# Jarvis73/PEMP

Hardware: AMD Instinct MI355X
Metric: episodes/sec (PEMP stage-1 eval step, PASCAL-5i-shaped 1-shot, ResNet-50) (higher is better)
Workload: dtype f32

## Files before the change

pemp_amd/build.py:

```python
import hashlib
import os
import subprocess
from concurrent.futures import ThreadPoolExecutor

HERE = os.path.dirname(os.path.abspath(__file__))
CSRC = os.path.join(HERE, "csrc")
OBJ = os.path.join(HERE, "_obj")
OUT = os.path.join(HERE, "libpemp_hip.so")
SOURCES = ("conv_igemm.hip", "conv_dma.hip", "conv_dma2.hip", "conv_panel.hip", "conv_stem_pool.hip", "conv_wgrad.hip", "train_ops.hip", "pool_misc.hip", "head.hip", "head_bwd.hip", "cedt.hip",
           "episode_io.hip", "dropout.hip", "cm_linear.hip", "pfenet.hip", "pfenet_bwd.hip", "canet.hip", "canet_bwd.hip", "rpmms.hip", "rpmms_bwd.hip")
FLAGS = ["-O3", "--offload-arch=gfx950", "-std=c++17", "-fPIC"]


def _headers():
    return [os.path.join(CSRC, f) for f in sorted(os.listdir(CSRC)) if f.endswith((".h", ".inc"))] + \
           [os.path.join(HERE, "..", "include", "pemp_hip.h")]


def csrc_digest():
    h = hashlib.sha1()
    for f in sorted(os.listdir(CSRC)):
        with open(os.path.join(CSRC, f), "rb") as fh:
            h.update(f.encode() + b"\0" + fh.read())
    with open(os.path.join(HERE, "..", "include", "pemp_hip.h"), "rb") as fh:
        h.update(fh.read())
    return h.hexdigest()[:12]


CONV_ENGINE = ("common.h", "conv_common.h", "conv_tiles.h", "conv_igemm.hip", "conv_dma.hip", "conv_dma2.hip", "conv_panel.hip", "conv_stem_pool.hip")


def conv_digest():
    h = hashlib.sha1()
    for f in CONV_ENGINE:
        with open(os.path.join(CSRC, f), "rb") as fh:
            h.update(f.encode() + b"\0" + fh.read())
    return h.hexdigest()[:12]


def needs_build():
    if not os.path.exists(OUT):
        return True
    t = os.path.getmtime(OUT)
    deps = [os.path.join(CSRC, f) for f in os.listdir(CSRC)] + [os.path.join(HERE, "..", "include", "pemp_hip.h")]
# ... 49 lines not shown
```

pemp_amd/csrc/conv_common.h:

```cpp
#pragma once
#include "common.h"

namespace pemp {

typedef __attribute__((ext_vector_type(16))) float f32x16;
typedef __attribute__((ext_vector_type(4))) float v4f;
typedef __attribute__((ext_vector_type(8))) __bf16 bf16x8;
typedef __attribute__((ext_vector_type(2))) unsigned int u32x2;

#define PEMP_CONV_BF16_IO 0x100u

__device__ __forceinline__ v4f load_quad(const float* base, size_t off, unsigned bf16) {
    if (!bf16) return *(const v4f*)(base + off);
    const u32x2 r = *(const u32x2*)((const unsigned short*)base + off);
    return v4f{__builtin_bit_cast(float, r.x << 16), __builtin_bit_cast(float, r.x & 0xFFFF0000u),
               __builtin_bit_cast(float, r.y << 16), __builtin_bit_cast(float, r.y & 0xFFFF0000u)};
}

__device__ __forceinline__ unsigned int bf16_bits(float f) {
    const unsigned int u = __builtin_bit_cast(unsigned int, f);
    if ((u & 0x7FFFFFFFu) > 0x7F800000u) return (u >> 16) | 0x40u;
    return (u + 0x7FFFu + ((u >> 16) & 1u)) >> 16;
}

// ... 300 lines not shown
int conv_dma2_hybrid_rows(int M, int Cout);
int launch_conv_dma2_bf16(int shape, const ConvArgs& a, hipStream_t st);
int launch_conv_dma2_db(int shape, ConvArgs a, void* ws, size_t ws_bytes, bool split, hipStream_t st);
struct SplitKPlan { int full, split, pieces; size_t ws_bytes; };
SplitKPlan conv_dma2_splitk_plan(int shape, const ConvArgs& a);
int launch_conv_dma2_splitk(int shape, ConvArgs a, void* ws, size_t ws_bytes, hipStream_t st);
int launch_conv_dma2_split3(int shape, ConvArgs a, void* ws, size_t ws_bytes, bool split, hipStream_t st);
int launch_conv_dma2_group_split3(int shape, ConvGroupArgs& g, hipStream_t st);
int launch_conv_dma2_split3_stats(int shape, const ConvArgs& a, hipStream_t st);
bool conv_dma2_split3_stats_shape(int shape);
int launch_conv_dma2_split3_persist(int shape, const ConvArgs& a, hipStream_t st);
bool conv_dma2_persist_out_split3(int shape);
int launch_conv_dma2_split3_pre(int shape, bool persistent, const ConvArgs& a, hipStream_t st);
bool conv_panel_supported(const ConvArgs& a);
int launch_conv_panel(int shape, const ConvArgs& a, hipStream_t st);
int conv_dma2_simds();
int pack_split3(const float* w, void* out, int cout, int kpad, hipStream_t st);
int launch_conv_stem_pool(const ConvArgs& a, hipStream_t st);
int conv_stem_pool_out(int i);

}
```

pemp_amd/csrc/conv_igemm.hip:

```cpp
#include "conv_tiles.h"

namespace pemp {


template <int BM, int BN, int WGM, bool STEM>
__global__ __launch_bounds__(256) void conv_igemm_kernel(ConvArgs a) {
    constexpr int WGN = 4 / WGM;
    constexpr int WM = BM / WGM, WN = BN / WGN;
    constexpr int TM = WM / 32, TN = WN / 32;
    constexpr int AL = BM / 32, BL = BN / 32;
    static_assert(TM >= 1 && TN >= 1, "wave tile");

    extern __shared__ __attribute__((aligned(16))) v4f smem[];
    v4f* As = smem;
    v4f* Bs = smem + 2 * 8 * BM;

    const int tid = threadIdx.x;
    const int lane = tid & 63;
    const int wave = tid >> 6;
    const int wm0 = (wave / WGN) * WM;
    const int wn0 = (wave % WGN) * WN;
    const int lr = lane & 31, lh = lane >> 5;

    const int ntn = a.Cout / BN;
// ... 292 lines not shown
                     "conv2d: PEMP_CONV_POOL3S2 needs PEMP_CONV_STEM4 with split3 weights (a tile id 41..49), no residual, no padding value");
        return launch_conv_stem_pool(a, (hipStream_t)stream);
    }
    PEMP_REQUIRE(tile != 33 && tile != 53, "conv2d: no split-K variant of the 64 x 64 tile");
    PEMP_REQUIRE(tile != 45 && tile != 55, "conv2d: no split3 form of the 128 x 64 8-wave tile");
    PEMP_REQUIRE(tile != 48, "conv2d: no persistent split3 form of the 128 x 128 4-wave tile");
    PEMP_REQUIRE(t.exists, "conv2d: unknown tile id %d", tile);
    hipStream_t st = (hipStream_t)stream;
    PEMP_REQUIRE(t.presplit == ((d->flags & PEMP_CONV_IN_SPLIT3) != 0), "conv2d: tile ids 146 / 149 and PEMP_CONV_IN_SPLIT3 come together (tile %d)", tile);
    if (t.presplit) {
        PEMP_REQUIRE(!stem && !ws && a.ntaps > 1 && a.ntaps <= 16 && a.ldx == a.Cin && !(d->flags & PEMP_CONV_SHIFT_PER_IMAGE),
                     "conv2d: tile %d takes convs of 2..16 taps with ldx == Cin, no per-image shift, no workspace", tile);
        PEMP_REQUIRE(conv_dma2_supported(a) && (long long)a.Cout * a.Kpad * 6 < (1ll << 31),
                     "conv2d: tile %d needs <= 32 taps and operands < 2 GiB (a padding value behind the activations)", tile);
        PEMP_REQUIRE_COUT("conv2d", t.shape, a.Cout);
        return launch_conv_dma2_split3_pre(t.shape, t.persistent, a, st);
    }
    if (t.family == TILE_SPLIT3) {
        PEMP_REQUIRE(!stem && conv_dma2_supported(a) && (long long)a.Cout * a.Kpad * 6 < (1ll << 31),
                     "conv2d: split3 tile %d needs a geometry of the buffer-addressed kernels (no stem, <= 32 taps, operands < 2 GiB)", tile);
        PEMP_REQUIRE_COUT("conv2d", t.shape, a.Cout);
        if (t.panel) {
            PEMP_REQUIRE(!ws && conv_panel_supported(a),
                         "conv2d: tile %d needs a 1x1 conv without padding, Kpad <= 256, no padding value / per-image shift / workspace, operands < 2 GiB", tile);
            return launch_conv_panel(t.shape, a, st);
        }
        if (t.persistent && (!out_split3 || conv_dma2_persist_out_split3(t.shape))) return launch_conv_dma2_split3_persist(t.shape, a, st);
        return launch_conv_dma2_split3(t.shape, a, ws, ws_bytes, t.splitk, st);
    }
    if (t.family == TILE_DMA2 && t.splitk) {
// ... 252 lines not shown
```

pemp_amd/csrc/conv_tiles.h:

```cpp
#pragma once
#include <initializer_list>
#include "conv_common.h"

namespace pemp {

struct TileShape { int bm, bn, wgm, nw, wgm3; };
inline constexpr TileShape kTileShapes[10] = {
    {0, 0, 0, 0, 0},
    {128, 128, 2, 4, 4},
    {128, 64, 2, 4, 4},
    {64, 64, 2, 4, 2},
    {128, 128, 4, 8, 4},
    {128, 64, 4, 8, 0},
    {256, 128, 4, 8, 8},
    {256, 256, 4, 8, 0},
    {32, 64, 2, 4, 0},
    {64, 64, 2, 4, 0},
};

template <int S, bool S3 = false>
struct Tile {
    static constexpr int BM = kTileShapes[S].bm, BN = kTileShapes[S].bn, NW = kTileShapes[S].nw;
    static constexpr int WGM = S3 ? kTileShapes[S].wgm3 : kTileShapes[S].wgm;
};
// ... 24 lines not shown
            if (shape == S) return f(Tile<S, Fam::s3>{});
        }
        return with_tile<Fam, S + 1>(shape, f);
    }
}

enum TileFamily { TILE_NONE = 0, TILE_IGEMM, TILE_DMA, TILE_DMA2, TILE_SPLIT3 };
struct TileId {
    int family;
    int shape;
    bool splitk;
    bool persistent;
    bool exists;
    bool panel;
    bool presplit;
};

inline TileId decode_tile(int id) {
    TileId t = {TILE_NONE, 0, false, false, false, false, false};
    const int decade = id / 10, s = id % 10;
    if (id == 146 || id == 149) {
        t.family = TILE_SPLIT3, t.shape = 6, t.exists = t.presplit = true, t.persistent = id == 149;
        return t;
    }
    if (decade == 7 && in_family<FamPanel>(s)) {
        t.family = TILE_SPLIT3, t.shape = s, t.exists = t.panel = true;
        return t;
    }
    if (id < 1 || id > 56 || s == 0) return t;
    t.shape = s;
    if (decade == 0) t.family = TILE_IGEMM, t.exists = in_family<FamIgemm>(s);
    else if (decade == 1) t.family = TILE_DMA, t.exists = in_family<FamFp32>(s);
    else if (decade == 2) t.family = TILE_DMA2, t.exists = true;
    else if (decade == 3) t.family = TILE_DMA2, t.splitk = true, t.exists = in_family<FamSplitK>(s);
    else if (decade == 4 && (s == 7 || s == 9)) t.family = TILE_SPLIT3, t.persistent = t.exists = true, t.shape = s == 7 ? 3 : 6;
    else if (decade == 4) t.family = TILE_SPLIT3, t.exists = in_family<FamSplit3>(s);
    else t.family = TILE_SPLIT3, t.splitk = true, t.exists = in_family<FamSplit3>(s) && in_family<FamSplitK>(s);
// ... 45 lines not shown
```

pemp_amd/ops.py:

```python
import ctypes as C
import collections
import functools
import json
import os

import torch

from . import _lib
from ._lib import ConvDesc, CONV_RELU, CONV_SHIFT_PER_IMAGE, CONV_STEM4, CONV_POOL3S2, CONV_OUT_SPLIT3, CONV_IN_SPLIT3, CONV_OUT_SPLIT3_ALSO


def _stream():
    return C.c_void_p(torch.cuda.current_stream().cuda_stream)


def _p(t):
    return C.c_void_p(t.data_ptr()) if t is not None else C.c_void_p(0)


def _chk_dev(*ts):
    for t in ts:
        if t is not None and (not t.is_cuda):
            raise _lib.PempHipError("pemp_amd ops need device (cuda/HIP) tensors; there is no CPU path")

# ... 32 lines not shown
           8: (32, 64),
           9: (64, 64)}
Tile = collections.namedtuple("Tile", "shape family splitk persistent_of")
SPLIT3_PERSISTENT = {47: 43, 49: 46}
TILES = {base + s: Tile(_SHAPES[s], family, base in (30, 50), None)
         for family, base, shapes in (("igemm", 0, (1, 2, 3)),
                                      ("dma", 10, range(1, 8)),
                                      ("dma2", 20, range(1, 10)),
                                      ("dma2", 30, (1, 2, 4, 5, 6, 7)),
                                      ("split3", 40, (1, 2, 3, 4, 6)),
                                      ("split3", 50, (1, 2, 4, 6)))
         for s in shapes}
TILES.update({t: TILES[of]._replace(persistent_of=of) for t, of in SPLIT3_PERSISTENT.items()})
TILES.update({70 + s: Tile(_SHAPES[s], "split3", False, None) for s in (1, 2)})
TILES.update({146: Tile(_SHAPES[6], "split3", False, None), 149: Tile(_SHAPES[6], "split3", False, 146)})
_NO_TILE = Tile(None, None, False, None)


def tile_shape(t):
    return TILES.get(t, _NO_TILE).shape


TILE_VARIANTS = {t: TILES[t].shape for t in (13, 14, 12, 11, 15, 3, 17, 16, 23, 24, 22, 21, 25, 27, 26, 28, 29)}
SPLIT3_TILES = (43, 42, 41, 44, 46, 47, 49)
SPLIT3_SPLITK_TILES = (51, 52, 54, 56)
SPLIT3_DEFAULT_TILE = 43
SPLIT3_PANEL_TILES = (71, 72)
SPLIT3_PANEL = os.environ.get("PEMP_SPLIT3_PANEL", "1") != "0"
SPLIT3_PRESPLIT_TILES = (146, 149)
SPLIT3_PRESPLIT = os.environ.get("PEMP_SPLIT3_PRESPLIT", "1") != "0"
AUTOTUNE = True
PICK_HOOK = None
SPLITK = os.environ.get("PEMP_CONV_SPLITK", "1") != "0"
DEFAULT_TILE = 13
_TILE_CACHE = {}
_TILE_CACHE_FILE = os.environ.get("PEMP_TILE_CACHE")
WGRAD_PICKS = {}
if _TILE_CACHE_FILE and os.path.exists(_TILE_CACHE_FILE):
    with open(_TILE_CACHE_FILE) as _f:
        for _k, _v in json.load(_f).items():
            _key = json.loads(_k)
            if _key and _key[0] == "wgrad":
                WGRAD_PICKS[tuple(_key[1:])] = tuple(_v) if isinstance(_v, list) else int(_v)
            else:
                _TILE_CACHE[tuple(_key)] = int(_v)
# ... 95 lines not shown
    best = min(top, key=lambda t: final[t])
    _TILE_CACHE[key] = best
    save_picks()
    return best


def _tile_bn(t):
    return TILES[t].shape[1]


def _panel_ok(p, n, ho, wo, ldx, ldy, ldr, h, w, pad_value, splitk, per_image_shift):
    lim = 1 << 31
    return (SPLIT3_PANEL and PICK_HOOK is None and p.kh == 1 and p.kw == 1 and p.pad == 0 and p.kpad <= 256 and p.cin % 32 == 0
            and pad_value is None and not splitk and not per_image_shift and n * h * w * ldx * 4 < lim
            and n * ho * wo * max(ldy, ldr) * 4 < lim)


def pack_split3(w):
    co, kpad = w.shape
    if w.dtype != torch.float32 or not w.is_contiguous() or kpad % 32:
        raise ValueError("pack_split3: a contiguous fp32 [Cout, Kpad] with Kpad % 32 == 0")
    out = torch.empty((co, kpad // 32, 3, 32), dtype=torch.bfloat16, device=w.device)
    _lib.check(_lib.load().pemp_pack_split3_bf16(_p(w), _p(out), co, kpad, _stream()), "pemp_pack_split3_bf16")
    return out


def hybrid_rows(n, ho, wo, cout):
    d = ConvDesc(n, ho, wo, 32, 32, ho, wo, cout, cout, 1, 1, 1, 0, 1, 0, 32, 0, 29)
    return int(_lib.load().pemp_conv2d_hybrid_rows(C.byref(d)))

# ... 60 lines not shown

def conv2d(x, p, out=None, residual=None, shift_override=None, per_image_shift=False, relu=None, tile=0,
           pad_value=None, splitk=False, dropblock=None, out_split3=False, x_split3=False, also_split3=None):
    if out_split3 or x_split3:
        what = "a pre-split output" if out_split3 else "a pre-split input"
        if p.w3 is None or p.stem:
            raise ValueError(f"conv2d: {what} needs a split3 layer (ConvParams.w3), not the fp32 chain or a stem")
        if splitk or dropblock is not None:
            raise ValueError(f"conv2d: {what} has no split-K / DropBlock form")
        if out_split3 and tile and (tile not in SPLIT3_TILES + SPLIT3_PRESPLIT_TILES):
            raise ValueError(f"conv2d: a pre-split output needs an unsplit split3 tile id, got {tile}")
        if x_split3 and (p.kh * p.kw == 1 or per_image_shift or p.cin % 32 or p.cout % 128):
            raise ValueError("conv2d: a pre-split input needs a multi-tap conv with Cin % 32 == 0 and Cout % 128 == 0, no per-image shift")
    if also_split3 is not None and (not x_split3 or out_split3 or residual is not None):
        raise ValueError("conv2d: a second, pre-split output needs a pre-split input (x_split3), no out_split3, no residual")
    if (tile in SPLIT3_PRESPLIT_TILES) != bool(x_split3) and (tile or not x_split3):
        raise ValueError(f"conv2d: the tile ids {SPLIT3_PRESPLIT_TILES} and x_split3 come together (tile {tile})")
    if x.dtype == torch.bfloat16 and not x_split3:
        return _conv2d_bf16(x, p, out, residual, shift_override, per_image_shift, relu, tile, pad_value)
    n, h, w, cin, ldx, ho, wo, out, ldy, ldr = _conv_geom("conv2d", x, p, out, residual, x_split3=x_split3, out_split3=out_split3)
    if also_split3 is not None and _split3_dims(also_split3, "also_split3") != (n, ho, wo, p.cout):
        raise ValueError(f"conv2d: also_split3 shape {tuple(also_split3.shape)} != {split3_shape(n, ho, wo, p.cout)}")
    lib = _lib.load()
    _chk_dev(x, p.w, out, residual, also_split3)
    if also_split3 is not None:
        residual = also_split3
    shift = p.shift if shift_override is None else shift_override
    if pad_value is not None:
        _chk_dev(pad_value)
        if x_split3:
            if tuple(pad_value.shape) != (cin // 32, 3, 32) or pad_value.dtype != torch.bfloat16 or not pad_value.is_contiguous():
                raise ValueError(f"conv2d: with x_split3, pad_value must be a contiguous bf16 [{cin // 32}, 3, 32] split vector")
# ... 45 lines not shown
            ws, ws_bytes = _splitk_ws(lib, d, x.device)
            _check_sk(lib, lib.pemp_conv2d_splitk_nhwc_f32(C.byref(d), _p(x), _p(pw), _p(out), _p(p.scale), _p(shift), _p(residual),
                                                           C.c_void_p(ws), ws_bytes, _stream()), ws, "pemp_conv2d_splitk_nhwc_f32")
        elif pad_value is None:
            _lib.check(lib.pemp_conv2d_nhwc_f32(C.byref(d), _p(x), _p(pw), _p(out), _p(p.scale), _p(shift),
                                                _p(residual), _stream()), "pemp_conv2d_nhwc_f32")
        else:
            _lib.check(lib.pemp_conv2d_padv_nhwc_f32(C.byref(d), _p(x), _p(pw), _p(out), _p(p.scale), _p(shift),
                                                     _p(residual), _p(pad_value), _stream()), "pemp_conv2d_padv_nhwc_f32")

    if tile == 0:
        key = (p.cin, p.cout, p.kh, p.kw, p.stride, p.pad, p.dil, (6 if dropblock is not None else 4) if splitk else int(p.stem) + (7 if dropblock is not None else 0),
               n, h, w, int(residual is not None and also_split3 is None), int(pad_value is not None)) + ((3,) if s3 else ())
        if x_split3 or out_split3:
            key += (146,) * int(x_split3) + (17,) * int(out_split3) + (64,) * int(also_split3 is not None)
            cands = lambda: _fits(list(SPLIT3_PRESPLIT_TILES if x_split3 else SPLIT3_TILES), p.cout)
        elif s3:
            panel = _panel_ok(p, n, ho, wo, ldx, ldy, ldr, h, w, pad_value, splitk, per_image_shift)
            if panel:
                key += (71,)
            cands = lambda: _fits(list(SPLIT3_TILES) + (list(SPLIT3_SPLITK_TILES) if splitk else []) +
                                  (list(SPLIT3_PANEL_TILES) if panel else []), p.cout)
        else:
            def cands():
                ids = list(GROUP_TILES if dropblock is not None else TILE_VARIANTS) + (list(SPLITK_TILES) if splitk else [])
                if 29 in ids and not (hybrid_rows(n, ho, wo, p.cout) and dma2_supported(x, p)):
                    ids.remove(29)
                return _fits(ids, p.cout)
        tile = _choose_tile(key, n * ho * wo, launch, cands,
                            SPLIT3_PRESPLIT_TILES[0] if x_split3 else SPLIT3_DEFAULT_TILE if s3 else DEFAULT_TILE + (10 if dropblock is not None else 0))
    launch(tile)
# ... 819 lines not shown
```

scratch/conv_trace_layers.py:

```python
import collections
import csv
import sys

trace, per_step = sys.argv[1], int(sys.argv[2])
steps = int(sys.argv[3]) if len(sys.argv) > 3 else 20
rows = sorted(csv.DictReader(open(trace)), key=lambda r: int(r["Start_Timestamp"]))
conv = [r for r in rows if any(k in r["Kernel_Name"] for k in ("conv_dma", "conv_igemm", "conv_stem_pool", "conv_panel"))][-steps * per_step:]
dur = lambda r: (int(r["End_Timestamp"]) - int(r["Start_Timestamp"])) / 1e3
pos = collections.defaultdict(list)
for i, r in enumerate(conv):
    pos[i % per_step].append(r)
print(f"conv launches per step {per_step}, steps {steps}: conv {sum(map(dur, conv)) / steps / 1e3:.3f} ms per step")
print(f"{'pos':>3} {'mean us':>9} {'grid':>8} {'wg':>4}  kernel")
for p in range(per_step):
    rs = pos[p]
    r = rs[-1]
    name = r["Kernel_Name"].split("(")[0].replace("void pemp::", "").replace("pemp::", "")
    g = r.get("Grid_Size", r.get("Grid_Size_X", "")); wg = r.get("Workgroup_Size", r.get("Workgroup_Size_X", ""))
    print(f"{p:>3} {sum(map(dur, rs)) / len(rs):9.1f} {g:>8} {wg:>4}  {name}")
```

scratch/s3_layers_bench.py:

```python
import argparse
import hashlib
import os
import sys

import torch

sys.path.insert(0, os.path.dirname(os.path.dirname(os.path.abspath(__file__))))
from pemp_amd import ops

UNSPLIT = (43, 42, 41, 44, 46, 47, 49)
SPLIT = (52, 51, 54, 56)
PANEL = ops.SPLIT3_PANEL_TILES
PRESPLIT = ops.SPLIT3_PRESPLIT_TILES
LAYERS = ((256, 1024, 1, 1, True, False), (512, 1024, 1, 1, False, False), (1024, 256, 1, 1, False, False),
          (256, 256, 3, 2, False, False), (128, 512, 1, 1, True, False), (1024, 512, 1, 1, False, False),
          (256, 256, 3, 2, False, True),
          (64, 256, 1, 1, True, False, 1, 101), (64, 256, 1, 1, False, False, 1, 101), (256, 512, 1, 1, False, False, 2, 101),
          (128, 128, 3, 1, False, False), (128, 128, 3, 1, False, False, 2, 101), (64, 64, 3, 1, False, False, 1, 101),
          (512, 128, 1, 1, False, False),
          (256, 256, 3, 12, False, True))


def timed(fn, reps, n=5):
    for _ in range(2):
        fn()
    e0, e1 = torch.cuda.Event(enable_timing=True), torch.cuda.Event(enable_timing=True)
    best, worst = 1e9, 0.0
    for _ in range(reps):
# ... 60 lines not shown
                continue
            run = lambda: ops.conv2d(x, prm, residual=res, pad_value=pad_value, out=out, tile=tile)
            run()
            same = torch.equal(out, ref)
            if tile in SPLIT:
                hashes.append(f"{tile}=" + ("43" if same else digest(out)))
            us, worst = timed(run, args.reps)
            mark = "" if same else (" ~" if tile in SPLIT else " !")
            cells.append(f"{tile}: {us:7.1f}..{worst:6.1f}us {fl / us / 1e6:5.1f}TF{mark}")
            if tile not in SPLIT and not same:
                hashes.append(f"{tile}=MISMATCH:{digest(out)}")
        if k > 1 and cout % 128 == 0:
            sbuf = torch.zeros((M + 4) * cin * 3, dtype=torch.bfloat16, device=dev)
            sbuf[:(M + 1) * cin * 3] = presplit(buf[:M + 1]).reshape(-1)
            xs, pvs = sbuf[:M * cin * 3].view(N, HW, HW, cin // 32, 3, 32), sbuf[M * cin * 3:(M + 1) * cin * 3].view(cin // 32, 3, 32)
            for tile in keep(PRESPLIT):
                run = lambda: ops.conv2d(xs, prm, residual=res, pad_value=pvs if padv else None, out=out, tile=tile, x_split3=True)
                run()
                same = torch.equal(out, ref)
                us, worst = timed(run, args.reps)
                cells.append(f"{tile}: {us:7.1f}..{worst:6.1f}us {fl / us / 1e6:5.1f}TF{'' if same else ' !'}")
            if not has_res:
                want = presplit(ref)
                outs = torch.empty_like(want)
                for tile in keep(PRESPLIT):
                    run = lambda: ops.conv2d(xs, prm, pad_value=pvs if padv else None, out=out, tile=tile, x_split3=True, also_split3=outs)
                    out.zero_()
                    run()
                    same = torch.equal(out, ref) and torch.equal(outs.view(torch.int16), want.view(torch.int16))
                    us, worst = timed(run, args.reps)
                    cells.append(f"{tile}+s: {us:7.1f}..{worst:6.1f}us{'' if same else ' !'}")
                del want, outs
            del sbuf, xs, pvs
        if k == 1 and not has_res:
            want = presplit(ref)
            outs = torch.empty_like(want)
            for tile in keep((43, 42, 41, 44, 46, 47, 49) if not args.ids else ()):
                if cout % ops._tile_bn(tile):
                    continue
                run = lambda: ops.conv2d(x, prm, out=outs, tile=tile, out_split3=True)
                run()
                same = torch.equal(outs.view(torch.int16), want.view(torch.int16))
                us, worst = timed(run, args.reps)
                cells.append(f"{tile}s: {us:7.1f}..{worst:6.1f}us{'' if same else ' !'}")
            del want, outs
        print(f"{name:>16} k{k} d{dil} res{int(has_res)} | " + " | ".join(cells), flush=True)
        print(f"{'':>16} hash " + " ".join(hashes), flush=True)
    print("(146 / 149: on the pre-split input; NNs: id NN writing a pre-split output, ! = not the split of id 43's;")
    print(" NNN+s: id NNN writing fp32 and the pre-split copy, ! = either differs)")
    print("(! = an unsplit id differs from id 43; ~ = a split-K id differs from id 43, expected where it splits)")


if __name__ == "__main__":
    main()
```

Before: 1485.

## Add row-staged 3x3 conv kernel reusing one activation stage across kw taps

Adds a new split3 conv kernel (tiles 246/249) for 3x3 stride-1 convs on pre-split bf16 input. It stages a contiguous band of up to 288 input rows per kernel row and reads the three kw taps from that same LDS stage via shifted indices, instead of loading one stage per tap. This is meant to cut global-to-LDS traffic and barriers per K step. The autotuner adds these tiles as candidates when the shape fits, at the cost of more LDS use and a more complex pipeline schedule.

After: 1506, median of 6. +1.4%, better.

```diff
diff --git a/pemp_amd/build.py b/pemp_amd/build.py
--- a/pemp_amd/build.py
+++ b/pemp_amd/build.py
@@ -7,7 +7,7 @@
 CSRC = os.path.join(HERE, "csrc")
 OBJ = os.path.join(HERE, "_obj")
 OUT = os.path.join(HERE, "libpemp_hip.so")
-SOURCES = ("conv_igemm.hip", "conv_dma.hip", "conv_dma2.hip", "conv_panel.hip", "conv_stem_pool.hip", "conv_wgrad.hip", "train_ops.hip", "pool_misc.hip", "head.hip", "head_bwd.hip", "cedt.hip",
+SOURCES = ("conv_igemm.hip", "conv_dma.hip", "conv_dma2.hip", "conv_panel.hip", "conv_row3.hip", "conv_stem_pool.hip", "conv_wgrad.hip", "train_ops.hip", "pool_misc.hip", "head.hip", "head_bwd.hip", "cedt.hip",
            "episode_io.hip", "dropout.hip", "cm_linear.hip", "pfenet.hip", "pfenet_bwd.hip", "canet.hip", "canet_bwd.hip", "rpmms.hip", "rpmms_bwd.hip")
 FLAGS = ["-O3", "--offload-arch=gfx950", "-std=c++17", "-fPIC"]
 
@@ -27,7 +27,7 @@
     return h.hexdigest()[:12]
 
 
-CONV_ENGINE = ("common.h", "conv_common.h", "conv_tiles.h", "conv_igemm.hip", "conv_dma.hip", "conv_dma2.hip", "conv_panel.hip", "conv_stem_pool.hip")
+CONV_ENGINE = ("common.h", "conv_common.h", "conv_tiles.h", "conv_igemm.hip", "conv_dma.hip", "conv_dma2.hip", "conv_panel.hip", "conv_row3.hip", "conv_stem_pool.hip")
 
 
 def conv_digest():
diff --git a/pemp_amd/csrc/conv_common.h b/pemp_amd/csrc/conv_common.h
--- a/pemp_amd/csrc/conv_common.h
+++ b/pemp_amd/csrc/conv_common.h
@@ -338,6 +338,8 @@
 int launch_conv_dma2_split3_pre(int shape, bool persistent, const ConvArgs& a, hipStream_t st);
 bool conv_panel_supported(const ConvArgs& a);
 int launch_conv_panel(int shape, const ConvArgs& a, hipStream_t st);
+bool conv_row3_supported(const ConvArgs& a);
+int launch_conv_row3(bool persistent, const ConvArgs& a, hipStream_t st);
 int conv_dma2_simds();
 int pack_split3(const float* w, void* out, int cout, int kpad, hipStream_t st);
 int launch_conv_stem_pool(const ConvArgs& a, hipStream_t st);
diff --git a/pemp_amd/csrc/conv_igemm.hip b/pemp_amd/csrc/conv_igemm.hip
--- a/pemp_amd/csrc/conv_igemm.hip
+++ b/pemp_amd/csrc/conv_igemm.hip
@@ -330,6 +330,12 @@
         PEMP_REQUIRE(conv_dma2_supported(a) && (long long)a.Cout * a.Kpad * 6 < (1ll << 31),
                      "conv2d: tile %d needs <= 32 taps and operands < 2 GiB (a padding value behind the activations)", tile);
         PEMP_REQUIRE_COUT("conv2d", t.shape, a.Cout);
+        if (t.row3) {
+            PEMP_REQUIRE(conv_row3_supported(a),
+                         "conv2d: tile %d unsupported: needs a 3x3 / stride 1 / pad == dil conv, the plain fp32 output without residual / padding value, "
+                         "and a stage of at most 288 rows (256 + 2 d + d ceil((255 + 2 d) / W))", tile);
+            return launch_conv_row3(t.persistent, a, st);
+        }
         return launch_conv_dma2_split3_pre(t.shape, t.persistent, a, st);
     }
     if (t.family == TILE_SPLIT3) {
diff --git a/pemp_amd/csrc/conv_row3.hip b/pemp_amd/csrc/conv_row3.hip
--- /dev/null
+++ b/pemp_amd/csrc/conv_row3.hip
@@ -0,0 +1,481 @@
+#include "conv_tiles.h"
+
+namespace pemp {
+
+typedef __attribute__((address_space(3))) void* lptr_t;
+
+constexpr int ROW3_BM = 256, ROW3_BN = 128, ROW3_NW = 8, ROW3_WGM = 4;
+constexpr int ROW3_SR = 288;
+constexpr int ROW3_AQ = ROW3_SR * 12, ROW3_BQ = ROW3_BN * 12;
+constexpr int ROW3_AL = (ROW3_AQ + ROW3_NW * 64 - 1) / (ROW3_NW * 64);
+constexpr int ROW3_BL = ROW3_BQ / (ROW3_NW * 64);
+constexpr int ROW3_SPARE = ROW3_AL * ROW3_NW * 64 - ROW3_AQ;
+static_assert(ROW3_BQ % (ROW3_NW * 64) == 0 && ROW3_SPARE % 64 == 0 && ROW3_SPARE < ROW3_NW * 64, "whole waves in the last A round");
+constexpr size_t row3_lds() { return (size_t)(2 * ROW3_AQ + 2 * ROW3_BQ + ROW3_SPARE) * sizeof(v4f); }
+static_assert(row3_lds() <= 160 * 1024, "LDS of a CU");
+
+constexpr int row3_a_tail(int ph) { return ph == 2 ? 3 : ph == 0 ? ROW3_AL - 3 : 0; }
+constexpr int row3_a_first(int ph) { return ph == 0 ? 3 : 0; }
+static_assert(row3_a_tail(0) + row3_a_tail(1) + row3_a_tail(2) == ROW3_AL, "a group's pieces over its window");
+constexpr int row3_behind(int ph) { return ph == 2 ? 0 : row3_a_tail((ph + 2) % 3); }
+constexpr int row3_behind_first() { return ROW3_BL + row3_a_tail(2); }
+
+__global__ __launch_bounds__(ROW3_NW * 64) __attribute__((amdgpu_waves_per_eu(2))) void conv_row3_kernel(ConvArgs a) {
+#if defined(__HIP_DEVICE_COMPILE__)
+    constexpr int BM = ROW3_BM, BN = ROW3_BN, NW = ROW3_NW, WGM = ROW3_WGM, WGN = NW / WGM;
+    constexpr int WM = BM / WGM, WN = BN / WGN, TM = WM / 32, TN = WN / 32;
+    constexpr int AL = ROW3_AL, BL = ROW3_BL;
+    constexpr int NMF = 6 * TM * TN, NDS = 3 * TM + 3 * TN;
+
+    extern __shared__ __attribute__((aligned(16))) v4f smem[];
+    v4f* As = smem;
+    v4f* Bs = smem + 2 * ROW3_AQ;
+    v4f* Sp = Bs + 2 * ROW3_BQ;
+
+    const int tid = threadIdx.x;
+    const int lane = tid & 63;
+    const int wave = __builtin_amdgcn_readfirstlane(tid >> 6);
+    const int wm0 = (wave / WGN) * WM, wn0 = (wave % WGN) * WN;
+    const int lr = lane & 31, lh = lane >> 5;
+
+    const int ntn = a.Cout / BN;
+    const int tile_id = xcd_tile_order(blockIdx.x, gridDim.x);
+    const int m0 = (tile_id / ntn) * BM, n0 = (tile_id % ntn) * BN;
+
+    const int d = a.dil, W = a.W, Wd = W + d;
+    const int f0 = m0 - d;
+    const int R0 = f0 >= 0 ? f0 / W : -((W - 1 - f0) / W);
+    const int c0 = f0 - R0 * W;
+    const int rowb = a.ldx * 6;
+    const __amdgpu_buffer_rsrc_t rx =
+        __builtin_amdgcn_make_buffer_rsrc((void*)((const char*)a.x - (ptrdiff_t)(d * W + d) * rowb), 0, 0x80000000u, 0x00020000);
+    const __amdgpu_buffer_rsrc_t rw = __builtin_amdgcn_make_buffer_rsrc((void*)a.w, 0, 0x80000000u, 0x00020000);
+
+    unsigned a_voff[AL], a_ok = 0, b_voff[BL];
+#pragma unroll
+    for (int i = 0; i < AL; ++i) {
+        const int q = i * NW * 64 + tid, srow = q / 12, pos = q - srow * 12;
+        const int src = (pos & ~3) | ((pos & 3) ^ ((srow >> 2) & 3));
+        const int t = srow + c0, rr = t / Wd, cc = t - rr * Wd;
+        const int f = (R0 + rr) * W + cc;
+        const bool pix = srow < ROW3_SR && cc < W && f >= 0 && f < a.M && f < m0 + BM + d;
+        const int h = pix ? (R0 + rr) % a.H : 0;
+        a_voff[i] = (unsigned)((f + d) * rowb + src * 16);
+#pragma unroll
+        for (int kh = 0; kh < 3; ++kh)
+            if (pix && (unsigned)(h + (kh - 1) * d) < (unsigned)a.H) a_ok |= 1u << (3 * i + kh);
+    }
+#pragma unroll
+    for (int i = 0; i < BL; ++i) {
+        const int q = i * NW * 64 + tid, row = q / 12, pos = q - row * 12;
+        const int src = (pos & ~3) | ((pos & 3) ^ ((row >> 2) & 3));
+        b_voff[i] = (unsigned)((n0 + row) * a.Kpad * 6 + src * 16);
+    }
+    const int taph = d * W * rowb;
+    const int NG = 3 * a.cin_steps, nkl = a.nk;
+
+#define PEMP_ROW3_DMA_A(i_, ab_, cb_, kh_, ok_)                                                                   \
+    do {                                                                                                          \
+        const int so_ = __builtin_amdgcn_readfirstlane((kh_) * taph + (cb_) * 192);                              \
+        const bool in_ = (((a_ok & (0u - (unsigned)(ok_))) >> (3 * (i_) + (kh_))) & 1u) != 0u;    \
+        v4f* dst_ = As + (ab_) * ROW3_AQ + (i_) * NW * 64 + wave * 64;                                            \
+        if ((i_) == AL - 1 && ROW3_SPARE) dst_ = wave * 64 < NW * 64 - ROW3_SPARE ? dst_ : Sp + (wave * 64 - (NW * 64 - ROW3_SPARE)); \
+        __builtin_amdgcn_raw_ptr_buffer_load_lds(rx, (lptr_t)dst_, 16, in_ ? a_voff[i_] : 0x80000000u, so_, 0, 0); \
+    } while (0)
+#define PEMP_ROW3_DMA_B(bb_, cb_, tap_, ok_)                                                                      \
+    do {                                                                                                          \
+        const int so_ = __builtin_amdgcn_readfirstlane(((tap_) * a.Cin + (cb_) * 32) * 6);                       \
+        _Pragma("unroll") for (int i = 0; i < BL; ++i)                                                            \
+            __builtin_amdgcn_raw_ptr_buffer_load_lds(rw, (lptr_t)(Bs + (bb_) * ROW3_BQ + i * NW * 64 + wave * 64), 16, \
+                                                     (ok_) ? b_voff[i] : 0x80000000u, so_, 0, 0);                 \
+    } while (0)
+
+    int aidx[TM][3][2];
+#pragma unroll
+    for (int mi = 0; mi < TM; ++mi) {
+        const int m = m0 + wm0 + mi * 32 + lr;
+        const int s = m - f0 + d * (m / W - R0);
+#pragma unroll
+        for (int kw = 0; kw < 3; ++kw) {
+            const int row = s + (kw - 1) * d, sw = (row >> 2) & 3;
+            aidx[mi][kw][0] = row * 12 + (lh ^ sw);
+            aidx[mi][kw][1] = row * 12 + ((2 + lh) ^ sw);
+        }
+    }
+    const int brow3 = (wn0 + lr) * 12, bsw3 = (lr >> 2) & 3;
+
+    f32x16 acc[TM][TN];
+#pragma unroll
+    for (int mi = 0; mi < TM; ++mi)
+#pragma unroll
+        for (int ni = 0; ni < TN; ++ni)
+#pragma unroll
+            for (int e = 0; e < 16; ++e) acc[mi][ni][e] = 0.f;
+    v4f aq3[2][TM][3], bf3[2][TN][3];
+
+#define PEMP_ROW3_READ(dst_, ab_, bb_, kw_, j_)                                                                   \
+    do {                                                                                                          \
+        const v4f* Ab_ = As + (ab_) * ROW3_AQ;                                                                    \
+        const v4f* Bb_ = Bs + (bb_) * ROW3_BQ;                                                                    \
+        const int pb_ = (2 * (j_) + lh) ^ bsw3;                                                                   \
+        _Pragma("unroll") for (int mi = 0; mi < TM; ++mi)                                                         \
+            _Pragma("unroll") for (int pl = 0; pl < 3; ++pl)                                                      \
+                aq3[dst_][mi][pl] = Ab_[aidx[mi][kw_][j_] + pl * 4];                                              \
+        _Pragma("unroll") for (int ni = 0; ni < TN; ++ni)                                                         \
+            _Pragma("unroll") for (int pl = 0; pl < 3; ++pl)                                                      \
+                bf3[dst_][ni][pl] = Bb_[brow3 + ni * 32 * 12 + pl * 4 + pb_];                                     \
+    } while (0)
+
+#define PEMP_ROW3_MMA(src_)                                                                                       \
+    do {                                                                                                          \
+        _Pragma("unroll") for (int mi = 0; mi < TM; ++mi) _Pragma("unroll") for (int ni = 0; ni < TN; ++ni) {     \
+            const bf16x8 ah_ = __builtin_bit_cast(bf16x8, aq3[src_][mi][0]);                                      \
+            const bf16x8 am_ = __builtin_bit_cast(bf16x8, aq3[src_][mi][1]);                                      \
+            const bf16x8 al_ = __builtin_bit_cast(bf16x8, aq3[src_][mi][2]);                                      \
+            const bf16x8 bh_ = __builtin_bit_cast(bf16x8, bf3[src_][ni][0]);                                      \
+            const bf16x8 bm_ = __builtin_bit_cast(bf16x8, bf3[src_][ni][1]);                                      \
+            const bf16x8 bl_ = __builtin_bit_cast(bf16x8, bf3[src_][ni][2]);                                      \
+            acc[mi][ni] = __builtin_amdgcn_mfma_f32_32x32x16_bf16(al_, bh_, acc[mi][ni], 0, 0, 0);                \
+            acc[mi][ni] = __builtin_amdgcn_mfma_f32_32x32x16_bf16(ah_, bl_, acc[mi][ni], 0, 0, 0);                \
+            acc[mi][ni] = __builtin_amdgcn_mfma_f32_32x32x16_bf16(am_, bm_, acc[mi][ni], 0, 0, 0);                \
+            acc[mi][ni] = __builtin_amdgcn_mfma_f32_32x32x16_bf16(am_, bh_, acc[mi][ni], 0, 0, 0);                \
+            acc[mi][ni] = __builtin_amdgcn_mfma_f32_32x32x16_bf16(ah_, bm_, acc[mi][ni], 0, 0, 0);                \
+            acc[mi][ni] = __builtin_amdgcn_mfma_f32_32x32x16_bf16(ah_, bh_, acc[mi][ni], 0, 0, 0);                \
+        }                                                                                                         \
+    } while (0)
+
+#define PEMP_ROW3_STEP(PH_, GG_, OKB_, OKA1_, OKA2_)                                                              \
+    do {                                                                                                          \
+        const int ab = (GG_) & 1, bb_ = ((GG_) + (PH_)) & 1;                                                      \
+        PEMP_ROW3_READ(1, ab, bb_, PH_, 1);                                                                       \
+        __builtin_amdgcn_sched_barrier(0);                                                                        \
+        PEMP_ROW3_MMA(0);                                                                                         \
+        __builtin_amdgcn_sched_barrier(0);                                                                        \
+         \
+        __builtin_amdgcn_s_waitcnt(0xC07F);              \
+        asm volatile("s_waitcnt vmcnt(%0) lgkmcnt(0)" ::"n"(row3_behind(PH_)) : "memory");                        \
+        __builtin_amdgcn_s_barrier();                                                        \
+        __builtin_amdgcn_sched_barrier(0);                                                                        \
+        if ((PH_) == 2) PEMP_ROW3_READ(0, ab ^ 1, bb_ ^ 1, 0, 0);                                                 \
+        else PEMP_ROW3_READ(0, ab, bb_ ^ 1, (PH_) + 1, 0);                                                        \
+        if ((PH_) == 0) PEMP_ROW3_DMA_B(bb_, cb, kh * 3 + 2, OKB_);                                               \
+        else PEMP_ROW3_DMA_B(bb_, cbn, khn * 3 + (PH_) - 1, OKB_);                                                \
+        _Pragma("unroll") for (int i = 0; i < row3_a_tail(PH_); ++i) {                                            \
+            if ((PH_) == 2) PEMP_ROW3_DMA_A(row3_a_first(PH_) + i, ab, cbn2, khn2, OKA2_);                        \
+            else PEMP_ROW3_DMA_A(row3_a_first(PH_) + i, ab ^ 1, cbn, khn, OKA1_);                                 \
+        }                                                                                                         \
+        PEMP_ROW3_MMA(1);                \
+        _Pragma("unroll") for (int k_ = 0; k_ < NMF; ++k_) {                                                      \
+            __builtin_amdgcn_sched_group_barrier(0x008, 1, 0);                                                    \
+            if (k_ < NDS) __builtin_amdgcn_sched_group_barrier(0x100, 1, 0);                                      \
+            else if (k_ < NDS + BL + row3_a_tail(PH_)) __builtin_amdgcn_sched_group_barrier(0x020, 1, 0);         \
+        }                                                                                                         \
+        __builtin_amdgcn_sched_barrier(0);                                                                        \
+    } while (0)
+    static_assert(NDS + BL + ROW3_AL <= NMF, "one LDS read / one DMA per MFMA slot");
+
+#pragma unroll
+    for (int i = 0; i < AL; ++i) PEMP_ROW3_DMA_A(i, 0, 0, 0, true);
+    PEMP_ROW3_DMA_B(0, 0, 0, true);
+    PEMP_ROW3_DMA_B(1, 0, 1, true);
+#pragma unroll
+    for (int i = 0; i < row3_a_tail(2); ++i) PEMP_ROW3_DMA_A(i, 1, 0, 1, true);
+    asm volatile("s_waitcnt vmcnt(%0)" ::"n"(row3_behind_first()) : "memory");
+    __builtin_amdgcn_s_barrier();
+    __builtin_amdgcn_sched_barrier(0);
+
+    PEMP_ROW3_READ(0, 0, 0, 0, 0);
+    int cb = 0, kh = 0;
+    for (int g = 0; g < NG; ++g) {
+        const int cbn = kh == 2 ? cb + 1 : cb, khn = kh == 2 ? 0 : kh + 1;
+        const int cbn2 = khn == 2 ? cbn + 1 : cbn, khn2 = khn == 2 ? 0 : khn + 1;
+        PEMP_ROW3_STEP(0, g, 3 * g + 2 < nkl, g + 1 < NG, false);
+        PEMP_ROW3_STEP(1, g, 3 * g + 3 < nkl, false, false);
+        PEMP_ROW3_STEP(2, g, 3 * g + 4 < nkl, false, g + 2 < NG);
+        cb = cbn;
+        kh = khn;
+    }
+
+    __builtin_amdgcn_s_waitcnt(0xC07F);
+    asm volatile("s_waitcnt vmcnt(0) lgkmcnt(0)" ::: "memory");
+    __builtin_amdgcn_s_barrier();
+    __builtin_amdgcn_sched_barrier(0);
+    static_assert(NW * 1024 * sizeof(float) <= 2 * ROW3_AQ * sizeof(v4f), "one 4 KB transpose patch per wave");
+    conv_epilogue_lds<TM, TN>(a, acc, (float*)smem + wave * 1024, m0 + wm0, n0 + wn0, lane);
+#endif
+}
+
+template <int TM, int TN>
+__device__ __forceinline__ void conv_row3_epilogue(const ConvArgs& a, f32x16 (&acc)[TM][TN], float* S, int m_base, int n_base, int lane,
+                                                   const v4f (&scv)[TN], const v4f (&shv)[TN]) {
+    const bool relu = a.flags & PEMP_CONV_RELU;
+    const int lr = lane & 31, lh = lane >> 5;
+    const int rr = lane >> 3, c4 = (lane & 7) * 4;
+#pragma unroll
+    for (int ni = 0; ni < TN; ++ni) {
+        const int n = n_base + ni * 32 + c4;
+        const v4f sc = scv[ni], sh = shv[ni];
+#pragma unroll
+        for (int mi = 0; mi < TM; ++mi) {
+#pragma unroll
+            for (int e = 0; e < 16; ++e) S[((e & 3) + 8 * (e >> 2) + 4 * lh) * 32 + lr] = acc[mi][ni][e];
+            asm volatile("s_waitcnt lgkmcnt(0)" ::: "memory");
+#pragma unroll
+            for (int i = 0; i < 4; ++i) {
+                const int row = rr + 8 * i;
+                const int m = m_base + mi * 32 + row;
+                const v4f v = *(const v4f*)(S + row * 32 + c4);
+                if (m < a.M) {
+                    const v4f add = sh;
+                    v4f o;
+                    o.x = __builtin_fmaf(v.x, sc.x, add.x);
+                    o.y = __builtin_fmaf(v.y, sc.y, add.y);
+                    o.z = __builtin_fmaf(v.z, sc.z, add.z);
+                    o.w = __builtin_fmaf(v.w, sc.w, add.w);
+                    if (relu) {
+                        o.x = fmaxf(o.x, 0.f);
+                        o.y = fmaxf(o.y, 0.f);
+                        o.z = fmaxf(o.z, 0.f);
+                        o.w = fmaxf(o.w, 0.f);
+                    }
+                    store_quad(a.y, (size_t)m * a.ldy + n, o, 0);
+                }
+            }
+            asm volatile("s_waitcnt lgkmcnt(0)" ::: "memory");
+        }
+    }
+}
+
+__global__ __launch_bounds__(ROW3_NW * 64) __attribute__((amdgpu_waves_per_eu(2))) void conv_row3p_kernel(ConvArgs a) {
+#if defined(__HIP_DEVICE_COMPILE__)
+    constexpr int BM = ROW3_BM, BN = ROW3_BN, NW = ROW3_NW, WGM = ROW3_WGM, WGN = NW / WGM;
+    constexpr int WM = BM / WGM, WN = BN / WGN, TM = WM / 32, TN = WN / 32;
+    constexpr int AL = ROW3_AL, BL = ROW3_BL;
+    constexpr int NMF = 6 * TM * TN, NDS = 3 * TM + 3 * TN;
+    constexpr int NST = TM * TN * 4;
+    static_assert(row3_behind_first() + NST <= 63, "vmcnt range");
+
+    extern __shared__ __attribute__((aligned(16))) v4f smem[];
+    v4f* As = smem;
+    v4f* Bs = smem + 2 * ROW3_AQ;
+    v4f* Sp = Bs + 2 * ROW3_BQ;
+
+    const int tid = threadIdx.x;
+    const int lane = tid & 63;
+    const int wave = __builtin_amdgcn_readfirstlane(tid >> 6);
+    const int wm0 = (wave / WGN) * WM, wn0 = (wave % WGN) * WN;
+    const int lr = lane & 31, lh = lane >> 5;
+
+    const int ntn = a.Cout / BN;
+    const int T = (a.M + BM - 1) / BM * ntn;
+    const int xcd = (int)blockIdx.x & 7, idx = (int)blockIdx.x >> 3;
+    const int q8 = T >> 3, r8 = T & 7;
+    const int t_first = xcd < r8 ? xcd * (q8 + 1) : r8 * (q8 + 1) + (xcd - r8) * q8;
+    const int t_cnt = q8 + (xcd < r8 ? 1 : 0);
+    const int gx = ((int)gridDim.x - xcd + 7) >> 3;
+    if (idx >= t_cnt) return;
+    int j = idx;
+    int m0 = ((t_first + j) / ntn) * BM, n0 = ((t_first + j) % ntn) * BN;
+
+    const int d = a.dil, W = a.W, Wd = W + d;
+    const int rowb = a.ldx * 6;
+    const __amdgpu_buffer_rsrc_t rx =
+        __builtin_amdgcn_make_buffer_rsrc((void*)((const char*)a.x - (ptrdiff_t)(d * W + d) * rowb), 0, 0x80000000u, 0x00020000);
+    const __amdgpu_buffer_rsrc_t rw = __builtin_amdgcn_make_buffer_rsrc((void*)a.w, 0, 0x80000000u, 0x00020000);
+
+    unsigned a_voff[AL], a_ok = 0, b_voff[BL];
+    auto a_offsets = [&](const int m0_, const bool ok_) {
+        const int f0 = m0_ - d;
+        const int R0 = f0 >= 0 ? f0 / W : -((W - 1 - f0) / W);
+        const int c0 = f0 - R0 * W;
+        a_ok = 0;
+#pragma unroll
+        for (int i = 0; i < AL; ++i) {
+            const int q = i * NW * 64 + tid, srow = q / 12, pos = q - srow * 12;
+            const int src = (pos & ~3) | ((pos & 3) ^ ((srow >> 2) & 3));
+            const int t = srow + c0, rr = t / Wd, cc = t - rr * Wd;
+            const int f = (R0 + rr) * W + cc;
+            const bool pix = ok_ && srow < ROW3_SR && cc < W && f >= 0 && f < a.M && f < m0_ + BM + d;
+            const int h = pix ? (R0 + rr) % a.H : 0;
+            a_voff[i] = (unsigned)((f + d) * rowb + src * 16);
+#pragma unroll
+            for (int kh = 0; kh < 3; ++kh)
+                if (pix && (unsigned)(h + (kh - 1) * d) < (unsigned)a.H) a_ok |= 1u << (3 * i + kh);
+        }
+    };
+    auto b_offsets = [&](const int n0_, const bool ok_) {
+#pragma unroll
+        for (int i = 0; i < BL; ++i) {
+            const int q = i * NW * 64 + tid, row = q / 12, pos = q - row * 12;
+            const int src = (pos & ~3) | ((pos & 3) ^ ((row >> 2) & 3));
+            b_voff[i] = ok_ ? (unsigned)((n0_ + row) * a.Kpad * 6 + src * 16) : 0x80000000u;
+        }
+    };
+    int aidx[TM][3][2];
+    auto reader = [&](const int m0_) {
+        const int f0 = m0_ - d;
+        const int R0 = f0 >= 0 ? f0 / W : -((W - 1 - f0) / W);
+#pragma unroll
+        for (int mi = 0; mi < TM; ++mi) {
+            const int m = m0_ + wm0 + mi * 32 + lr;
+            const int s = m - f0 + d * (m / W - R0);
+#pragma unroll
+            for (int kw = 0; kw < 3; ++kw) {
+                const int row = s + (kw - 1) * d, sw = (row >> 2) & 3;
+                aidx[mi][kw][0] = row * 12 + (lh ^ sw);
+                aidx[mi][kw][1] = row * 12 + ((2 + lh) ^ sw);
+            }
+        }
+    };
+    a_offsets(m0, true);
+    b_offsets(n0, true);
+    const int taph = d * W * rowb;
+    const int NG = 3 * a.cin_steps, ncb = a.cin_steps;
+    const int brow3 = (wn0 + lr) * 12, bsw3 = (lr >> 2) & 3;
+    const int c4_ = (lane & 7) * 4;
+    v4f aq3[2][TM][3], bf3[2][TN][3];
+
+#pragma unroll
+    for (int i = 0; i < AL; ++i) PEMP_ROW3_DMA_A(i, 0, 0, 0, true);
+    PEMP_ROW3_DMA_B(0, 0, 0, true);
+    PEMP_ROW3_DMA_B(1, 0, 1, true);
+#pragma unroll
+    for (int i = 0; i < row3_a_tail(2); ++i) PEMP_ROW3_DMA_A(i, 1, 0, 1, true);
+    asm volatile("s_waitcnt vmcnt(%0)" ::"n"(row3_behind_first()) : "memory");
+    __builtin_amdgcn_s_barrier();
+    __builtin_amdgcn_sched_barrier(0);
+
+    int gg = 0;
+    int cb = 0, kh = 0;
+    for (;;) {
+        f32x16 acc[TM][TN];
+#pragma unroll
+        for (int mi = 0; mi < TM; ++mi)
+#pragma unroll
+            for (int ni = 0; ni < TN; ++ni)
+#pragma unroll
+                for (int e = 0; e < 16; ++e) acc[mi][ni][e] = 0.f;
+        const int jn = j + gx;
+        const bool more = jn < t_cnt;
+        const int m0n = more ? ((t_first + jn) / ntn) * BM : m0, n0n = more ? ((t_first + jn) % ntn) * BN : n0;
+        reader(m0);
+
+        PEMP_ROW3_READ(0, gg & 1, gg & 1, 0, 0);
+#define PEMP_ROW3_NEXT_GROUPS()                                                                                   \
+        int cbn = kh == 2 ? cb + 1 : cb;                                                                          \
+        const int khn = kh == 2 ? 0 : kh + 1;                                                                     \
+        cbn = cbn == ncb ? 0 : cbn;                                                                               \
+        int cbn2 = khn == 2 ? cbn + 1 : cbn;                                                                      \
+        const int khn2 = khn == 2 ? 0 : khn + 1;                                                                  \
+        cbn2 = cbn2 == ncb ? 0 : cbn2
+        for (int g = 0; g < NG - 1; ++g, ++gg) {
+            PEMP_ROW3_NEXT_GROUPS();
+            PEMP_ROW3_STEP(0, gg, true, true, true);
+            if (g == NG - 2) a_offsets(m0n, more);
+            PEMP_ROW3_STEP(1, gg, true, true, true);
+            PEMP_ROW3_STEP(2, gg, true, true, true);
+            cb = cbn;
+            kh = khn;
+        }
+        const int abl = gg & 1;
+        {
+            PEMP_ROW3_NEXT_GROUPS();
+            PEMP_ROW3_STEP(0, gg, true, true, true);
+            b_offsets(n0n, more);
+            PEMP_ROW3_STEP(1, gg, true, true, true);
+            PEMP_ROW3_READ(1, abl, (gg + 2) & 1, 2, 1);
+            __builtin_amdgcn_sched_barrier(0);
+            PEMP_ROW3_MMA(0);
+            __builtin_amdgcn_sched_barrier(0);
+            __builtin_amdgcn_s_waitcnt(0xC07F);
+            asm volatile("s_waitcnt lgkmcnt(0)" ::: "memory");
+            __builtin_amdgcn_s_barrier();
+            __builtin_amdgcn_sched_barrier(0);
+            PEMP_ROW3_MMA(1);
+            __builtin_amdgcn_sched_barrier(0);
+            cb = cbn;
+            kh = khn;
+            (void)cbn2;
+            (void)khn2;
+            ++gg;
+        }
+#undef PEMP_ROW3_NEXT_GROUPS
+        v4f scv[TN], shv[TN];
+#pragma unroll
+        for (int ni = 0; ni < TN; ++ni) {
+            const int n = n0 + wn0 + ni * 32 + c4_;
+            scv[ni] = a.scale ? *(const v4f*)(a.scale + n) : v4f{1.f, 1.f, 1.f, 1.f};
+            shv[ni] = a.shift ? *(const v4f*)(a.shift + n) : v4f{0.f, 0.f, 0.f, 0.f};
+        }
+        static_assert(NW * 256 <= ROW3_AQ, "one 4 KB transpose patch per wave inside ONE stage buffer");
+        conv_row3_epilogue<TM, TN>(a, acc, (float*)(As + abl * ROW3_AQ + wave * 256), m0 + wm0, n0 + wn0, lane, scv, shv);
+        if (!more) {
+            asm volatile("s_waitcnt vmcnt(0)" ::: "memory");
+            break;
+        }
+
+        __builtin_amdgcn_s_barrier();
+        PEMP_ROW3_DMA_B((gg + 1) & 1, 0, 1, true);
+#pragma unroll
+        for (int i = 0; i < row3_a_tail(2); ++i) PEMP_ROW3_DMA_A(i, (gg + 1) & 1, 0, 1, true);
+        constexpr int VF = row3_behind_first() + NST, VP = row3_behind_first();
+        if (m0 + wm0 + WM <= a.M) {
+            __builtin_amdgcn_s_waitcnt((VF & 15) | 0x0F70 | ((VF >> 4) << 14));
+            asm volatile("s_waitcnt vmcnt(%0)" ::"n"(VF) : "memory");
+        } else {
+            __builtin_amdgcn_s_waitcnt((VP & 15) | 0x0F70 | ((VP >> 4) << 14));
+            asm volatile("s_waitcnt vmcnt(%0)" ::"n"(VP) : "memory");
+        }
+        __builtin_amdgcn_s_barrier();
+        __builtin_amdgcn_sched_barrier(0);
+        j = jn;
+        m0 = m0n;
+        n0 = n0n;
+    }
+#endif
+}
+#undef PEMP_ROW3_STEP
+#undef PEMP_ROW3_MMA
+#undef PEMP_ROW3_READ
+#undef PEMP_ROW3_DMA_B
+#undef PEMP_ROW3_DMA_A
+
+static long long row3_stage_rows(int W, int d) { return ROW3_BM + 2 * d + (long long)d * ((ROW3_BM - 1 + 2 * d + W - 1) / W); }
+
+bool conv_row3_supported(const ConvArgs& a) {
+    if (!(a.flags & PEMP_CONV_IN_SPLIT3) || (a.flags & (PEMP_CONV_OUT_SPLIT3 | PEMP_CONV_OUT_SPLIT3_ALSO | PEMP_CONV_SHIFT_PER_IMAGE | PEMP_CONV_STEM4 | PEMP_CONV_BF16_IO)))
+        return false;
+    if (a.res || a.padv || a.stats || a.rowmask || a.sk_S > 1 || a.sk_ws || a.bm_first) return false;
+    if (a.KH != 3 || a.KW != 3 || a.stride != 1 || a.pad != a.dil || a.ldx != a.Cin || a.Cin % 32 || a.Cout % ROW3_BN) return false;
+    if (a.Kpad != 9 * a.Cin || a.nk != 9 * a.cin_steps) return false;
+    if (row3_stage_rows(a.W, a.dil) > ROW3_SR) return false;
+    return conv_dma2_supported(a) && (long long)a.Cout * a.Kpad * 6 < (1ll << 31);
+}
+
+int launch_conv_row3(bool persistent, const ConvArgs& a, hipStream_t st) {
+    if (!conv_row3_supported(a)) {
+        set_error("conv split3 row3: unsupported (needs a 3x3 / stride 1 / pad == dil conv on pre-split input, plain fp32 output without residual / "
+                  "padding value / per-image shift / workspace, Cout %% 128 == 0, 256 + 2 d + d ceil((255 + 2 d) / W) <= %d stage rows)", ROW3_SR);
+        return -1;
+    }
+    const int tiles = cdiv(a.M, ROW3_BM) * (a.Cout / ROW3_BN);
+    if (!persistent) return launch_with_lds(conv_row3_kernel, tiles, ROW3_NW * 64, row3_lds(), st, a, "conv_row3");
+    static int occ = 0;
+    if (!occ) {
+        const int rc = allow_lds(conv_row3p_kernel, row3_lds());
+        if (rc) return rc;
+        int v = 0;
+        hipError_t e = hipOccupancyMaxActiveBlocksPerMultiprocessor(&v, (const void*)conv_row3p_kernel, ROW3_NW * 64, row3_lds());
+        if (e != hipSuccess || v <= 0) {
+            set_error("conv split3 row3 persistent: occupancy query failed (%s, %d blocks)", hipGetErrorString(e), v);
+            return -1;
+        }
+        occ = v;
+    }
+    long long grid = (long long)occ * (conv_dma2_simds() / 4);
+    if (grid < 8) grid = 8;
+    if (grid > tiles) grid = tiles;
+    return launch_with_lds(conv_row3p_kernel, (int)grid, ROW3_NW * 64, row3_lds(), st, a, "conv_row3/persistent");
+}
+
+}
diff --git a/pemp_amd/csrc/conv_tiles.h b/pemp_amd/csrc/conv_tiles.h
--- a/pemp_amd/csrc/conv_tiles.h
+++ b/pemp_amd/csrc/conv_tiles.h
@@ -62,13 +62,14 @@
     bool exists;
     bool panel;
     bool presplit;
+    bool row3;
 };
 
 inline TileId decode_tile(int id) {
-    TileId t = {TILE_NONE, 0, false, false, false, false, false};
+    TileId t = {TILE_NONE, 0, false, false, false, false, false, false};
     const int decade = id / 10, s = id % 10;
-    if (id == 146 || id == 149) {
-        t.family = TILE_SPLIT3, t.shape = 6, t.exists = t.presplit = true, t.persistent = id == 149;
+    if (id == 146 || id == 149 || id == 246 || id == 249) {
+        t.family = TILE_SPLIT3, t.shape = 6, t.exists = t.presplit = true, t.persistent = id % 10 == 9, t.row3 = id > 200;
         return t;
     }
     if (decade == 7 && in_family<FamPanel>(s)) {
diff --git a/pemp_amd/ops.py b/pemp_amd/ops.py
--- a/pemp_amd/ops.py
+++ b/pemp_amd/ops.py
@@ -70,6 +70,7 @@
 TILES.update({t: TILES[of]._replace(persistent_of=of) for t, of in SPLIT3_PERSISTENT.items()})
 TILES.update({70 + s: Tile(_SHAPES[s], "split3", False, None) for s in (1, 2)})
 TILES.update({146: Tile(_SHAPES[6], "split3", False, None), 149: Tile(_SHAPES[6], "split3", False, 146)})
+TILES.update({246: Tile(_SHAPES[6], "split3", False, None), 249: Tile(_SHAPES[6], "split3", False, 246)})
 _NO_TILE = Tile(None, None, False, None)
 
 
@@ -85,6 +86,9 @@
 SPLIT3_PANEL = os.environ.get("PEMP_SPLIT3_PANEL", "1") != "0"
 SPLIT3_PRESPLIT_TILES = (146, 149)
 SPLIT3_PRESPLIT = os.environ.get("PEMP_SPLIT3_PRESPLIT", "1") != "0"
+SPLIT3_ROW3_TILES = (246, 249)
+SPLIT3_ROW3 = os.environ.get("PEMP_SPLIT3_ROW3", "1") != "0"
+ROW3_STAGE_ROWS = 288
 AUTOTUNE = True
 PICK_HOOK = None
 SPLITK = os.environ.get("PEMP_CONV_SPLITK", "1") != "0"
@@ -210,6 +214,16 @@
     return (SPLIT3_PANEL and PICK_HOOK is None and p.kh == 1 and p.kw == 1 and p.pad == 0 and p.kpad <= 256 and p.cin % 32 == 0
             and pad_value is None and not splitk and not per_image_shift and n * h * w * ldx * 4 < lim
             and n * ho * wo * max(ldy, ldr) * 4 < lim)
+
+
+def row3_stage_rows(w, dil):
+    return 256 + 2 * dil + dil * ((255 + 2 * dil + w - 1) // w)
+
+
+def _row3_ok(p, w, residual, pad_value, out_split3, also_split3, per_image_shift):
+    return (SPLIT3_ROW3 and (p.kh, p.kw, p.stride) == (3, 3, 1) and p.pad == p.dil and residual is None
+            and pad_value is None and not out_split3 and also_split3 is None and not per_image_shift
+            and row3_stage_rows(w, p.dil) <= ROW3_STAGE_ROWS)
 
 
 def pack_split3(w):
@@ -300,8 +314,8 @@
             raise ValueError("conv2d: a pre-split input needs a multi-tap conv with Cin % 32 == 0 and Cout % 128 == 0, no per-image shift")
     if also_split3 is not None and (not x_split3 or out_split3 or residual is not None):
         raise ValueError("conv2d: a second, pre-split output needs a pre-split input (x_split3), no out_split3, no residual")
-    if (tile in SPLIT3_PRESPLIT_TILES) != bool(x_split3) and (tile or not x_split3):
-        raise ValueError(f"conv2d: the tile ids {SPLIT3_PRESPLIT_TILES} and x_split3 come together (tile {tile})")
+    if (tile in SPLIT3_PRESPLIT_TILES + SPLIT3_ROW3_TILES) != bool(x_split3) and (tile or not x_split3):
+        raise ValueError(f"conv2d: the tile ids {SPLIT3_PRESPLIT_TILES + SPLIT3_ROW3_TILES} and x_split3 come together (tile {tile})")
     if x.dtype == torch.bfloat16 and not x_split3:
         return _conv2d_bf16(x, p, out, residual, shift_override, per_image_shift, relu, tile, pad_value)
     n, h, w, cin, ldx, ho, wo, out, ldy, ldr = _conv_geom("conv2d", x, p, out, residual, x_split3=x_split3, out_split3=out_split3)
@@ -377,7 +391,11 @@
                n, h, w, int(residual is not None and also_split3 is None), int(pad_value is not None)) + ((3,) if s3 else ())
         if x_split3 or out_split3:
             key += (146,) * int(x_split3) + (17,) * int(out_split3) + (64,) * int(also_split3 is not None)
-            cands = lambda: _fits(list(SPLIT3_PRESPLIT_TILES if x_split3 else SPLIT3_TILES), p.cout)
+            row3 = bool(x_split3) and _row3_ok(p, w, residual, pad_value, out_split3, also_split3, per_image_shift)
+            if row3:
+                key += (246,)
+            cands = lambda: _fits(list(SPLIT3_PRESPLIT_TILES if x_split3 else SPLIT3_TILES) +
+                                  (list(SPLIT3_ROW3_TILES) if row3 and PICK_HOOK is None else []), p.cout)
         elif s3:
             panel = _panel_ok(p, n, ho, wo, ldx, ldy, ldr, h, w, pad_value, splitk, per_image_shift)
             if panel:
diff --git a/scratch/conv_trace_layers.py b/scratch/conv_trace_layers.py
--- a/scratch/conv_trace_layers.py
+++ b/scratch/conv_trace_layers.py
@@ -5,7 +5,7 @@
 trace, per_step = sys.argv[1], int(sys.argv[2])
 steps = int(sys.argv[3]) if len(sys.argv) > 3 else 20
 rows = sorted(csv.DictReader(open(trace)), key=lambda r: int(r["Start_Timestamp"]))
-conv = [r for r in rows if any(k in r["Kernel_Name"] for k in ("conv_dma", "conv_igemm", "conv_stem_pool", "conv_panel"))][-steps * per_step:]
+conv = [r for r in rows if any(k in r["Kernel_Name"] for k in ("conv_dma", "conv_igemm", "conv_stem_pool", "conv_panel", "conv_row3"))][-steps * per_step:]
 dur = lambda r: (int(r["End_Timestamp"]) - int(r["Start_Timestamp"])) / 1e3
 pos = collections.defaultdict(list)
 for i, r in enumerate(conv):
diff --git a/scratch/s3_layers_bench.py b/scratch/s3_layers_bench.py
--- a/scratch/s3_layers_bench.py
+++ b/scratch/s3_layers_bench.py
@@ -12,6 +12,7 @@
 SPLIT = (52, 51, 54, 56)
 PANEL = ops.SPLIT3_PANEL_TILES
 PRESPLIT = ops.SPLIT3_PRESPLIT_TILES
+ROW3 = ops.SPLIT3_ROW3_TILES
 LAYERS = ((256, 1024, 1, 1, True, False), (512, 1024, 1, 1, False, False), (1024, 256, 1, 1, False, False),
           (256, 256, 3, 2, False, False), (128, 512, 1, 1, True, False), (1024, 512, 1, 1, False, False),
           (256, 256, 3, 2, False, True),
@@ -102,8 +103,10 @@
             sbuf = torch.zeros((M + 4) * cin * 3, dtype=torch.bfloat16, device=dev)
             sbuf[:(M + 1) * cin * 3] = presplit(buf[:M + 1]).reshape(-1)
             xs, pvs = sbuf[:M * cin * 3].view(N, HW, HW, cin // 32, 3, 32), sbuf[M * cin * 3:(M + 1) * cin * 3].view(cin // 32, 3, 32)
-            for tile in keep(PRESPLIT):
+            row3 = ROW3 if k == 3 and stride == 1 and not has_res and not padv and ops.row3_stage_rows(HW, dil) <= ops.ROW3_STAGE_ROWS else ()
+            for tile in keep(PRESPLIT + row3):
                 run = lambda: ops.conv2d(xs, prm, residual=res, pad_value=pvs if padv else None, out=out, tile=tile, x_split3=True)
+                out.zero_()
                 run()
                 same = torch.equal(out, ref)
                 us, worst = timed(run, args.reps)
@@ -134,7 +137,7 @@
             del want, outs
         print(f"{name:>16} k{k} d{dil} res{int(has_res)} | " + " | ".join(cells), flush=True)
         print(f"{'':>16} hash " + " ".join(hashes), flush=True)
-    print("(146 / 149: on the pre-split input; NNs: id NN writing a pre-split output, ! = not the split of id 43's;")
+    print("(146 / 149 / 246 / 249: on the pre-split input; NNs: id NN writing a pre-split output, ! = not the split of id 43's;")
     print(" NNN+s: id NNN writing fp32 and the pre-split copy, ! = either differs)")
     print("(! = an unsplit id differs from id 43; ~ = a split-K id differs from id 43, expected where it splits)")
 
```
